# chechaohp/gan-ode

Measured on AMD Instinct MI355X. Metric: generated videos/sec (16-frame clips), higher is better.
Workload: dtype f32

## Files before the change

### gan-ode_amd/_lib.py

```python
from __future__ import annotations

import ctypes as C
import os

_HERE = os.path.dirname(os.path.abspath(__file__))
LIB_PATH = os.path.join(_HERE, "lib", "libgode.so")

i32, i64, f32, ptr = C.c_int32, C.c_int64, C.c_float, C.c_void_p
cint, u32, u64 = C.c_int, C.c_uint32, C.c_uint64

ACT_NONE, ACT_RELU, ACT_LRELU, ACT_TANH_OUT = 0, 1, 2, 3
EPI_RAW, EPI_TANH = 0, 1
FPROP, DGRAD = 0, 1
OP_IGEMM, OP_WGRAD, OP_BN_FINALIZE, OP_BN_BWD, OP_ODE_FWD, OP_ODE_BWD, OP_BCE, OP_ADAM, OP_PACK = range(1, 10)
OP_ODERNN_FWD, OP_ODERNN_BWD, OP_BN_APPLY, OP_COL2IM = 10, 11, 12, 13
OP_SDE_FWD, OP_SDE_BWD = 14, 15
OP_CDE_FWD, OP_CDE_BWD = 16, 17
OP_WGAN = 18
OP_GRU_FWD, OP_GRU_BWD = 19, 20
OP_DNOISE = 21
OP_CATEG, OP_CE = 22, 23
OP_CHSTATS, OP_CBN_EMBED, OP_CBN_EMBED_BWD, OP_CBN_APPLY, OP_CBN_BWD, OP_GRES_OUT, OP_GRES_OUT_BWD, OP_SN_FWD, OP_SN_BWD = range(24, 33)
REC_ADAM_NOISE = -1
ODE_NPARAM = 2672
ODERNN_NPARAM = 2176
SDE_NPARAM = 3216
CDE_NPARAM = 7536
CDE_MAX_N = 4096
# ... 4 lines not shown
class ConvGeom(C.Structure):
    _fields_ = [(n, i32) for n in "N Ci Co Di Hi Wi Do Ho Wo kd kh kw sd sh sw pd ph pw".split()]

    def key(self):
        return tuple(getattr(self, n) for n, _ in self._fields_)


class _Op(C.Structure):
    """An op of gode_run (a GODE_OPS row of gode.h): a subclass names its kind and its `int FN(const op*, stream)` entry
    point once; _STRUCTS, the prototypes, EXPORTS and run_one's dispatch all follow from the subclasses."""


class IgemmOp(_Op):
    _fields_ = [("g", ConvGeom), ("dir", i32), ("act", i32), ("epilogue", i32), ("tile", i32), ("src", ptr),
                ("wpack", ptr), ("out", ptr), ("scale", ptr), ("shift", ptr), ("stats", ptr), ("gs", i64 * 5),
                ("work", ptr), ("groups", i32), ("pad3_", i32)]
    KIND, FN = OP_IGEMM, "gode_igemm"


class WgradOp(_Op):
    _fields_ = [("g", ConvGeom), ("act", i32), ("xform_on_y", i32), ("splits", i32), ("accumulate", i32),
                ("x", ptr), ("y", ptr), ("scale", ptr), ("shift", ptr), ("work", ptr), ("dw", ptr),
                ("co_perm", ptr), ("co_canon", i64), ("xs", i64 * 5)]
    KIND, FN = OP_WGRAD, "gode_wgrad"


class BnFinalizeOp(_Op):
    _fields_ = [("stats", ptr), ("rows", i32), ("ncols", i32), ("C", i32), ("count", i64), ("gamma", ptr),
                ("beta", ptr), ("running_mean", ptr), ("running_var", ptr), ("num_batches_tracked", ptr),
                ("mean", ptr), ("invstd", ptr), ("scale", ptr), ("shift", ptr), ("momentum", f32), ("eps", f32),
                ("training", i32), ("pad_", i32), ("groups", i32), ("rows0", i32), ("nseg", i32), ("order", i32),
# ... 337 lines not shown
```

### gan-ode_amd/csrc/conv_geom.h

```cpp
#pragma once
#include <stdint.h>
#include "../../include/gode.h"

#if defined(__HIPCC__)
#define GODE_HD __host__ __device__ inline
#else
#define GODE_HD inline
#endif

#define GODE_MAX_PHASES 8

struct PhaseGeom {
  int32_t Md, Mh, Mw;
  int32_t M;
  int32_t Td, Th, Tw;
  int32_t K;
  int32_t Kp;
  int32_t Od, Oh, Ow;
  int32_t Pd, Ph, Pw;
  int32_t kd0, kh0, kw0;
  int32_t row0;
  int32_t img0;
  int64_t w_off;
};

struct IgemmGeom {
  int32_t nphase;
  int32_t Cg;
  int32_t Ncols;
  int32_t Sd, Sh, Sw;
  int32_t J;
  int32_t Gd, Gh, Gw;
  int32_t OSd, OSh, OSw;
  int32_t Xd, Xh, Xw;
  int32_t kstep_d, kstep_h, kstep_w;
  int32_t fullk;
  PhaseGeom ph[GODE_MAX_PHASES];
};

GODE_HD int gode_ceil_div(int a, int b) { return (a + b - 1) / b; }

inline int gode_build_igemm_geom(const gode_conv_geom& g, int dir, IgemmGeom* out) {
  IgemmGeom& G = *out;
  G.fullk = 0;
  if (g.N <= 0 || g.Ci <= 0 || g.Co <= 0) return GODE_E_SHAPE;
  if ((g.Di + 2 * g.pd - g.kd) / g.sd + 1 != g.Do || (g.Hi + 2 * g.ph - g.kh) / g.sh + 1 != g.Ho ||
      (g.Wi + 2 * g.pw - g.kw) / g.sw + 1 != g.Wo)
    return GODE_E_SHAPE;
  if (dir == GODE_FPROP) {
    G.nphase = 1; G.Cg = g.Ci; G.Ncols = g.Co;
    G.Sd = g.sd; G.Sh = g.sh; G.Sw = g.sw; G.J = 1;
    G.Gd = g.Di; G.Gh = g.Hi; G.Gw = g.Wi;
    G.OSd = G.OSh = G.OSw = 1;
    G.Xd = g.Do; G.Xh = g.Ho; G.Xw = g.Wo;
    G.kstep_d = G.kstep_h = G.kstep_w = 1;
    PhaseGeom& p = G.ph[0];
    p.Md = g.Do; p.Mh = g.Ho; p.Mw = g.Wo; p.M = g.N * p.Md * p.Mh * p.Mw;
    p.Td = g.kd; p.Th = g.kh; p.Tw = g.kw; p.K = p.Td * p.Th * p.Tw * G.Cg; p.Kp = (p.K + 3) & ~3;
    p.Od = -g.pd; p.Oh = -g.ph; p.Ow = -g.pw; p.Pd = p.Ph = p.Pw = 0;
    p.kd0 = p.kh0 = p.kw0 = 0; p.row0 = 0; p.img0 = 0; p.w_off = 0;
    return 0;
  }
  if (dir != GODE_DGRAD) return GODE_E_ARG;
  if (g.Do == 1 && g.Ho == 1 && g.Wo == 1 && g.pd == 0 && g.ph == 0 && g.pw == 0 && g.Di == g.kd &&
      g.Hi == g.kh && g.Wi == g.kw && g.kd * g.kh * g.kw > 1) {
    G.fullk = 1; G.nphase = 1; G.Cg = g.Co; G.Ncols = g.kd * g.kh * g.kw * g.Ci;
    G.Sd = G.Sh = G.Sw = 1; G.J = 1; G.Gd = G.Gh = G.Gw = 1;
    G.OSd = G.OSh = G.OSw = 1; G.Xd = G.Xh = G.Xw = 1;
    G.kstep_d = G.kstep_h = G.kstep_w = 1;
    PhaseGeom& p = G.ph[0];
    p.Md = p.Mh = p.Mw = 1; p.M = g.N; p.Td = p.Th = p.Tw = 1; p.K = G.Cg; p.Kp = (p.K + 3) & ~3;
    p.Od = p.Oh = p.Ow = 0; p.Pd = p.Ph = p.Pw = 0; p.kd0 = p.kh0 = p.kw0 = 0; p.row0 = 0; p.img0 = 0; p.w_off = 0;
    return 0;
  }
  if (g.sd * g.sh * g.sw > GODE_MAX_PHASES) return GODE_E_SHAPE;
  G.Cg = g.Co; G.Ncols = g.Ci;
  G.Sd = G.Sh = G.Sw = 1; G.J = -1;
  G.Gd = g.Do; G.Gh = g.Ho; G.Gw = g.Wo;
  G.OSd = g.sd; G.OSh = g.sh; G.OSw = g.sw;
  G.Xd = g.Di; G.Xh = g.Hi; G.Xw = g.Wi;
  G.kstep_d = g.sd; G.kstep_h = g.sh; G.kstep_w = g.sw;
  int np = 0; int64_t woff = 0;
  for (int fd = 0; fd < g.sd; ++fd)
    for (int fh = 0; fh < g.sh; ++fh)
      for (int fw = 0; fw < g.sw; ++fw) {
        PhaseGeom& p = G.ph[np++];
        const int phi[3] = {fd, fh, fw};
        const int X[3] = {g.Di, g.Hi, g.Wi}, s[3] = {g.sd, g.sh, g.sw}, k[3] = {g.kd, g.kh, g.kw},
                  pad[3] = {g.pd, g.ph, g.pw};
        int Mx[3], T[3], O[3], k0[3];
// ... 3 lines not shown
          k0[a] = r;
          T[a] = k[a] > r ? (k[a] - r + s[a] - 1) / s[a] : 0;
          O[a] = (phi[a] + pad[a] - r) / s[a];
        }
        p.Md = Mx[0]; p.Mh = Mx[1]; p.Mw = Mx[2]; p.M = g.N * Mx[0] * Mx[1] * Mx[2];
        p.Td = T[0]; p.Th = T[1]; p.Tw = T[2]; p.K = T[0] * T[1] * T[2] * G.Cg; p.Kp = (p.K + 3) & ~3;
        p.Od = O[0]; p.Oh = O[1]; p.Ow = O[2]; p.Pd = fd; p.Ph = fh; p.Pw = fw;
        p.kd0 = k0[0]; p.kh0 = k0[1]; p.kw0 = k0[2];
        p.row0 = 0; p.img0 = 0; p.w_off = woff;
        woff += (int64_t)G.Ncols * p.Kp;
      }
  G.nphase = np;
  return 0;
}

inline int64_t gode_pack_floats(const IgemmGeom& G) {
  int64_t t = 0;
  for (int i = 0; i < G.nphase; ++i) t += (int64_t)G.Ncols * G.ph[i].Kp;
  return t;
}

GODE_HD int64_t gode_w_index(const gode_conv_geom& g, int co, int ci, int kd, int kh, int kw) {
  return ((((int64_t)co * g.Ci + ci) * g.kd + kd) * g.kh + kh) * g.kw + kw;
}

GODE_HD int64_t gode_pack_source(const gode_conv_geom& g, int dir, const IgemmGeom& G, const PhaseGeom& p, int n,
                                 int k, const int32_t* co_perm) {
  if (k >= p.K) return -1;
  int co, ci, kd, kh, kw;
  if (G.fullk) {
    const int tapn = n / g.Ci;
    ci = n - tapn * g.Ci; co = k;
    kd = tapn / (g.kh * g.kw); kh = (tapn / g.kw) % g.kh; kw = tapn % g.kw;
// ... 12 lines not shown
```

### gan-ode_amd/csrc/igemm.hip

```cpp
#include <stdlib.h>
#include "common.h"
#include "conv_geom.h"

int gode_launch_conv_patch_fprop(const gode_igemm_op* op, const int64_t* gs, hipStream_t st);

struct IgemmArgs {
  IgemmGeom G;
  const float* src;
  const float* w;
  float* out;
  const float* scale;
  const float* shift;
  float* stats;
  int32_t gsN, gsD, gsH, gsW, gsC;
  int32_t act, epilogue;
  int32_t MB, NB, xcd_mode;
  int32_t tapskip, dmajor;
  int32_t stagger;
  int32_t ksplit, slabs_per_split;
  float* work;
  int32_t out_numel;
  int32_t stats_rows;
  uint32_t src_bytes, w_bytes;
};

__device__ __forceinline__ void igemm_block_id(const IgemmArgs& a, int& mblk, int& nblk, int& phase, int& split) {
  const int MB = a.MB, NC = a.NB * a.G.nphase;
  split = blockIdx.x / (MB * NC);
  const int id = blockIdx.x - split * (MB * NC);
  int combo;
  if (a.xcd_mode == 1) {
    const int x = id & 7, j = id >> 3;
    if ((NC & 7) == 0) { combo = x + 8 * (j / MB); mblk = j % MB; }
    else { const int parts = 8 / NC; combo = x % NC; mblk = j * parts + x / NC; }
  } else if (a.xcd_mode == 2) {
    const int x = id & 7, j = id >> 3;
    combo = j % NC; mblk = (j / NC) * 8 + x;
  } else if (a.xcd_mode == 3) {
    const int x = id & 7, j = id >> 3;
    combo = j % NC; mblk = x * (MB >> 3) + j / NC;
  } else {
// ... 952 lines not shown
      int k = (int)((1152 + t64 / 2) / t64);
      if (k < 1) k = 1;
      while (k > 1 && (min_slabs / k < 8 || out_bytes * k > 192e6)) --k;
      best_tile = TILE_64x64; best_k = k;
    }
  }
  *tile_out = best_tile;
  sp_out->positions = positions;
  sp_out->ksplit = 1; sp_out->slabs_per_split = 0;
  if (best_k > 1) {
    sp_out->slabs_per_split = gode_ceil_div(max_slabs, best_k);
    sp_out->ksplit = gode_ceil_div(max_slabs, sp_out->slabs_per_split);
  }
}

static int prepare(const gode_igemm_op* op, IgemmArgs* A, int* tile, int* max_mblk, int* rows, SplitPlan* sp, int* rows0 = nullptr) {
  int rc = gode_build_igemm_geom(op->g, op->dir, &A->G);
  if (rc) return rc;
  const bool grouped = op->groups == 2;
  if (grouped) {
    if (op->dir != GODE_FPROP || op->g.N % 2 != 0 || A->G.nphase != 1) return GODE_E_ARG;
    A->G.ph[1] = A->G.ph[0];
    A->G.ph[0].M /= 2; A->G.ph[1].M = A->G.ph[0].M; A->G.ph[1].img0 = op->g.N / 2;
    A->G.nphase = 2;
  } else if (op->groups != 0 && op->groups != 1) return GODE_E_ARG;
  static const char* menv = getenv("GODE_IGEMM_MODEL");
  static const bool sweeping = getenv("GODE_IGEMM_SWEEP") != nullptr;
  const char* fenv = sweeping ? getenv("GODE_IGEMM_FORCE") : nullptr;
  int ftile = 0, fk = 0;
  if (fenv && sscanf(fenv, "%d,%d", &ftile, &fk) == 2 && op->tile == 0 && fast_geometry(A->G) && A->G.Ncols > 4 &&
      strides_allow_vec(op, A->G)) {
    int max_slabs = 0;
    for (int i = 0; i < A->G.nphase; ++i) if ((A->G.ph[i].K >> 5) > max_slabs) max_slabs = A->G.ph[i].K >> 5;
    *tile = ftile;
    sp->positions = op->g.N * A->G.Xd * A->G.Xh * A->G.Xw; sp->ksplit = 1; sp->slabs_per_split = 0;
    if (fk > 1) { sp->slabs_per_split = gode_ceil_div(max_slabs, fk); sp->ksplit = gode_ceil_div(max_slabs, sp->slabs_per_split); }
  } else if (op->tile == 0 && fast_geometry(A->G) && A->G.Ncols > 4 && strides_allow_vec(op, A->G) && (!menv || atoi(menv) != 0)) {
    choose_fast(op, A->G, tile, sp);
  } else {
  *tile = pick_tile_split_aware(op->g, A->G, op->tile);
  *sp = plan_split(op, A->G, *tile);
  }
  if (grouped && sp->ksplit > 1 && (sp->positions / 2) % SPLITK_ROWS != 0) {
    sp->ksplit = 1; sp->slabs_per_split = 0;
  }
  const int bm = tile_bm(*tile);
  int r0 = 0, mx = 0;
  for (int i = 0; i < A->G.nphase; ++i) {
    A->G.ph[i].row0 = r0;
    const int mb = gode_ceil_div(A->G.ph[i].M, bm);
    r0 += mb;
    if (mb > mx) mx = mb;
  }
  *max_mblk = mx;
  *rows = sp->ksplit > 1 ? gode_ceil_div(sp->positions, SPLITK_ROWS) : r0;
  if (rows0) *rows0 = !grouped ? *rows : (sp->ksplit > 1 ? *rows / 2 : A->G.ph[1].row0);
// ... 1 lines not shown
}

extern "C" int gode_igemm_stats_rows0(const gode_igemm_op* op) {
  IgemmArgs A; int tile, mx, rows, rows0; SplitPlan sp;
  int rc = prepare(op, &A, &tile, &mx, &rows, &sp, &rows0);
  return rc ? rc : rows0;
}

extern "C" double gode_igemm_model_cycles(const gode_igemm_op* op) {
  if (!op || op->groups == 2 || op->tile != 0) return -1.0;
  IgemmArgs A;
  if (gode_build_igemm_geom(op->g, op->dir, &A.G)) return -1.0;
  static const char* menv = getenv("GODE_IGEMM_MODEL");
  if (!fast_geometry(A.G) || A.G.Ncols <= 4 || !strides_allow_vec(op, A.G) || (menv && atoi(menv) == 0)) return -1.0;
  int tile; SplitPlan sp; double cyc = -1.0;
  choose_fast(op, A.G, &tile, &sp, &cyc);
  return cyc;
}

extern "C" int gode_igemm_stats_segments(const gode_igemm_op* op, int32_t split_images, int32_t* seg) {
  if (!op || !seg || op->groups == 2 || split_images <= 0 || split_images >= op->g.N) return GODE_E_ARG;
  IgemmArgs A; int tile, mx, rows; SplitPlan sp;
  int rc = prepare(op, &A, &tile, &mx, &rows, &sp);
  if (rc) return rc;
  if (sp.ksplit > 1) {
    const int64_t per_img = (int64_t)A.G.Xd * A.G.Xh * A.G.Xw;
    const int64_t b = (int64_t)split_images * per_img;
    if (b % SPLITK_ROWS != 0) return GODE_E_SHAPE;
    seg[0] = 0; seg[1] = (int32_t)(b / SPLITK_ROWS); seg[2] = rows;
    return 1;
  }
  const int bm = tile_bm(tile);
  for (int i = 0; i < A.G.nphase; ++i) {
    const PhaseGeom& P = A.G.ph[i];
    const int64_t per_img = (int64_t)P.Md * P.Mh * P.Mw;
    const int64_t b = (int64_t)split_images * per_img;
// ... 36 lines not shown
    static const char* xenv = getenv("GODE_IGEMM_XCD");
    const int force = xenv ? atoi(xenv) : -1;
    const int64_t wbytes = gode_pack_floats(A.G) * 4;
    const bool ok1 = (NC % 8 == 0) || (NC < 8 && 8 % NC == 0 && MB % (8 / NC) == 0);
    const bool ok2 = MB % 8 == 0;
    const int64_t images = (int64_t)A.out_numel / ((int64_t)A.G.Xd * A.G.Xh * A.G.Xw * A.G.Ncols);
    const int64_t in_bytes = images * A.G.Gd * A.G.Gh * A.G.Gw * A.G.Cg * 4;
    int mode = ok2 ? (wbytes * 8 < 3 * in_bytes ? 3 : 0) : 0;
    if (A.dmajor > 0) mode = ok2 ? 2 : (ok1 ? 1 : 0);
    if (force == 0) mode = 0;
    if (force == 1 && ok1) mode = 1;
    if (force == 2 && ok2) mode = 2;
    if (force == 3 && ok2) mode = 3;
    A.xcd_mode = mode;
    dim3 g1(MB * NC * sp.ksplit);
    const bool has_xf = A.scale != nullptr || A.act != GODE_ACT_NONE;
    static const char* genv = getenv("GODE_IGEMM_GLDS");
    const bool glds = (genv ? atoi(genv) != 0 : true) && A.src_bytes != 0 && A.w_bytes != 0;
    if (!has_xf && glds && !double_buf) {
      if (A.tapskip) hipLaunchKernelGGL((igemm_fast_kernel<WM, WN, TM, TN, 3, false>), g1, block, 0, st, A);
      else hipLaunchKernelGGL((igemm_fast_kernel<WM, WN, TM, TN, 2, false>), g1, block, 0, st, A);
    } else if (double_buf) {
      if (has_xf) hipLaunchKernelGGL((igemm_fast_kernel<WM, WN, TM, TN, 1, true>), g1, block, 0, st, A);
      else hipLaunchKernelGGL((igemm_fast_kernel<WM, WN, TM, TN, 1, false>), g1, block, 0, st, A);
    } else {
      if (has_xf) hipLaunchKernelGGL((igemm_fast_kernel<WM, WN, TM, TN, 0, true>), g1, block, 0, st, A);
      else hipLaunchKernelGGL((igemm_fast_kernel<WM, WN, TM, TN, 0, false>), g1, block, 0, st, A);
    }
    if (sp.ksplit > 1) {
      GODE_LAUNCH_CHECK();
// ... 28 lines not shown
  }
  int64_t span = 1 + (int64_t)(op->g.N - 1) * gs[0] + (int64_t)(G.Gd - 1) * gs[1] + (int64_t)(G.Gh - 1) * gs[2] +
                 (int64_t)(G.Gw - 1) * gs[3] + (int64_t)(G.Cg - 1) * gs[4];
  int64_t outn = (int64_t)op->g.N * G.Xd * G.Xh * G.Xw * G.Ncols;
  for (int i = 0; i < 5; ++i) if (gs[i] < 0) return GODE_E_ARG;
  if (span >= (1ll << 31) || outn >= (1ll << 31)) return GODE_E_SHAPE;
  if (op->src && op->wpack && op->out && ((uintptr_t)op->wpack % 16) == 0) {
    const int pr = gode_launch_conv_patch_fprop(op, gs, (hipStream_t)stream);
    if (pr != 0) return pr < 0 ? pr : 0;
  }
  A.src = op->src; A.w = op->wpack; A.out = op->out; A.scale = op->scale; A.shift = op->shift; A.stats = op->stats;
  A.gsN = (int)gs[0]; A.gsD = (int)gs[1]; A.gsH = (int)gs[2]; A.gsW = (int)gs[3]; A.gsC = (int)gs[4];
  A.act = op->act; A.epilogue = op->epilogue;
  A.stagger = 0;
  A.dmajor = 0;
  A.tapskip = igemm_wants_tapskip(op, G);
  if (A.tapskip) A.dmajor = op->g.N;
  A.stats_rows = rows;
  A.src_bytes = span * 4 < (1ll << 31) ? (uint32_t)(span * 4) : 0u;
  A.w_bytes = gode_pack_floats(G) * 4 < (1ll << 31) ? (uint32_t)(gode_pack_floats(G) * 4) : 0u;
  A.work = op->work; A.out_numel = (int32_t)outn; A.ksplit = 1; A.slabs_per_split = 0; A.MB = 0; A.NB = 0; A.xcd_mode = 0;
  if ((op->scale == nullptr) != (op->shift == nullptr)) return GODE_E_ARG;
  const bool vec = gs[4] == 1 && (G.Cg % 4) == 0 && (gs[0] % 4) == 0 && (gs[1] % 4) == 0 && (gs[2] % 4) == 0 &&
                   (gs[3] % 4) == 0 && ((uintptr_t)op->src % 16) == 0 &&
                   (op->scale == nullptr || ((uintptr_t)op->scale % 16 == 0 && (uintptr_t)op->shift % 16 == 0));
  if (((uintptr_t)op->wpack % 16) != 0) return GODE_E_ARG;
  hipStream_t st = (hipStream_t)stream;
  if (op->groups != 2) {
    int maxM = 0, minK = 1 << 30; bool kp_ok = true;
    for (int i = 0; i < G.nphase; ++i) {
      if (G.ph[i].M > maxM) maxM = G.ph[i].M;
// ... 60 lines not shown
  const int32_t* co_perm;
};

__global__ void pack_kernel(const PackArgs a) {
  const PhaseGeom& P = a.G.ph[blockIdx.z];
  const int64_t total = (int64_t)a.G.Ncols * P.Kp;
  for (int64_t i = (int64_t)blockIdx.x * blockDim.x + threadIdx.x; i < total; i += (int64_t)gridDim.x * blockDim.x) {
    const int n = (int)(i / P.Kp), k = (int)(i - (int64_t)n * P.Kp);
    const int64_t src = gode_pack_source(a.g, a.dir, a.G, P, n, k, a.co_perm);
    a.wp[P.w_off + i] = src >= 0 ? a.w[src] : 0.f;
  }
}

extern "C" int64_t gode_pack_size(const gode_conv_geom* g, int dir) {
  IgemmGeom G;
  int rc = gode_build_igemm_geom(*g, dir, &G);
  return rc ? rc : gode_pack_floats(G);
}

#define PACK_BATCH 8
struct PackPhase { int32_t Th, Tw, K, Kp, kd0, kh0, kw0, pad_; int64_t w_off, total; };
struct PackEntry {
  const float* w; float* wp; const int32_t* co_perm;
  int32_t nphase, Cg, fullk, dir, ks_d, ks_h, ks_w, Ci, kd, kh, kw, Co;
  PackPhase ph[GODE_MAX_PHASES];
};
struct PackBatch { PackEntry e[PACK_BATCH]; };
static_assert(sizeof(PackBatch) <= 4096, "kernel-argument budget");

__global__ void __launch_bounds__(256) pack_batch_kernel(const PackBatch b) {
  const PackEntry& E = b.e[blockIdx.z];
  if ((int)blockIdx.y >= E.nphase) return;
  const PackPhase& P = E.ph[blockIdx.y];
  const int taps = E.kd * E.kh * E.kw;
  for (int64_t i = (int64_t)blockIdx.x * 256 + threadIdx.x; i < P.total; i += (int64_t)gridDim.x * 256) {
    const int n = (int)(i / P.Kp), k = (int)(i - (int64_t)n * P.Kp);
    float v = 0.f;
    if (k < P.K) {
      int co, ci, kd, kh, kw;
      if (E.fullk) {
// ... 42 lines not shown
    const int co_l = tid & (PACK_T - 1), ci_l = tid >> 4;
    for (int p = 0; p < E.nphase; ++p) {
      const PackPhase& P = E.ph[p];
      float* dst = E.wp + P.w_off + (int64_t)(ci0 + ci_l) * P.Kp + co0 + co_l;
      int j = 0;
      for (int kd = P.kd0; kd < E.kd; kd += E.ks_d)
        for (int kh = P.kh0; kh < E.kh; kh += E.ks_h)
          for (int kw = P.kw0; kw < E.kw; kw += E.ks_w, ++j) {
            const int t = (kd * E.kh + kh) * E.kw + kw;
            if (t >= t0 && t < t0 + TT) dst[(int64_t)j * E.Cg] = brick[co_l * CS + ci_l * 33 + (t - t0)];
          }
    }
  }
}

static bool pack_tileable(const PackEntry& E) {
  const int taps = E.kd * E.kh * E.kw;
  if (E.co_perm || E.fullk || taps < 4 || taps > 64 || (taps & (taps - 1)) != 0 || E.Ci % PACK_T != 0 || E.Co % PACK_T != 0) return false;
  for (int i = 0; i < E.nphase; ++i) if (E.ph[i].K != E.ph[i].Kp) return false;
  return true;
}

extern "C" int gode_pack_batch_(const gode_pack_op* const* ops, int n, void* stream) {
  for (int at = 0; at < n; at += PACK_BATCH) {
    PackBatch B;
    const int cnt = n - at < PACK_BATCH ? n - at : PACK_BATCH;
    int64_t mx = 0;
    for (int e = 0; e < cnt; ++e) {
      const gode_pack_op* op = ops[at + e];
      if (!op || !op->w || !op->wpack) return GODE_E_ARG;
      IgemmGeom G;
      const int rc = gode_build_igemm_geom(op->g, op->dir, &G);
      if (rc) return rc;
      PackEntry& E = B.e[e];
      E.w = op->w; E.wp = op->wpack; E.co_perm = op->co_perm;
      E.nphase = G.nphase; E.Cg = G.Cg; E.fullk = G.fullk; E.dir = op->dir;
      E.ks_d = G.kstep_d; E.ks_h = G.kstep_h; E.ks_w = G.kstep_w;
      E.Ci = op->g.Ci; E.kd = op->g.kd; E.kh = op->g.kh; E.kw = op->g.kw; E.Co = op->g.Co;
// ... 14 lines not shown
        const int taps = E.kd * E.kh * E.kw, TT = taps < 32 ? taps : 32;
        const int t = (E.Ci / PACK_T) * (E.Co / PACK_T) * (taps / TT);
        if (t > tiles) tiles = t;
        T.e[nt++] = E;
      } else {
        for (int i = 0; i < E.nphase; ++i) if (E.ph[i].total > mr) mr = E.ph[i].total;
        R.e[nr++] = E;
      }
    }
    if (nt > 0) {
      hipLaunchKernelGGL(pack_tile_kernel, dim3(tiles, 1, nt), dim3(256), 0, (hipStream_t)stream, T);
      GODE_LAUNCH_CHECK();
    }
    if (nr > 0 && mr > 0) {
      int blocks = (int)((mr + 1023) / 1024); if (blocks > 512) blocks = 512; if (blocks < 1) blocks = 1;
      hipLaunchKernelGGL(pack_batch_kernel, dim3(blocks, GODE_MAX_PHASES, nr), dim3(256), 0, (hipStream_t)stream, R);
      GODE_LAUNCH_CHECK();
    }
  }
  return 0;
}

extern "C" int gode_pack_weights(const gode_conv_geom* g, int dir, const float* w, float* wpack, const int32_t* co_perm,
                                 int32_t co_canon, void* stream) {
  (void)co_canon;
  if (!g || !w || !wpack) return GODE_E_ARG;
  PackArgs A;
  int rc = gode_build_igemm_geom(*g, dir, &A.G);
  if (rc) return rc;
  A.g = *g; A.dir = dir; A.w = w; A.wp = wpack; A.co_perm = co_perm;
  int64_t mx = 0;
  for (int i = 0; i < A.G.nphase; ++i) { int64_t t = (int64_t)A.G.Ncols * A.G.ph[i].Kp; if (t > mx) mx = t; }
  if (mx == 0) return 0;
  int blocks = (int)((mx + 255) / 256); if (blocks > 2048) blocks = 2048;
  hipLaunchKernelGGL(pack_kernel, dim3(blocks, 1, A.G.nphase), dim3(256), 0, (hipStream_t)stream, A);
  GODE_LAUNCH_CHECK();
  return 0;
}
```

### gan-ode_amd/engine.py

```python
from __future__ import annotations

import ctypes as C
from dataclasses import dataclass
from typing import List, Optional, Sequence

import numpy as np
import torch

from . import _lib as L


def make_geom(N, Ci, Co, xi, yo, k, s, p) -> L.ConvGeom:
    return L.ConvGeom(N, Ci, Co, xi[0], xi[1], xi[2], yo[0], yo[1], yo[2], k[0], k[1], k[2], s[0], s[1], s[2],
                      p[0], p[1], p[2])


def conv_out(i, k, s, p):
    return (i + 2 * p - k) // s + 1


def dptr(t: Optional[torch.Tensor]):
    return None if t is None else t.data_ptr()


# ... 64 lines not shown
        self.busy = False
        self.generation = 0
        self._fwd_training = True
        self.pack_cache = pack_cache if pack_cache is not None else {}
        lib = L.lib()
        f32 = dict(dtype=torch.float32, device=device)
        self.x_in = torch.zeros(specs[0].in_dims(), **f32) if owns_input else None
        self.x0n = torch.empty(specs[0].in_dims(), **f32) if specs[0].noise else None
        self.y = [torch.empty(s.out_dims(), **f32) for s in specs[:-1]]
        self.a = [torch.empty(s.out_dims(), **f32) if self._materialize(l) else None for l, s in enumerate(specs[:-1])]
        self.out_dims = specs[-1].out_dims()
        self.wpack_f, self.wpack_b = [], [None] * self.nl
        self.stats, self.stat_rows = [], []
        self.mean, self.invstd, self.scale, self.shift = [], [], [], []
        self._two_f, self._two_b, self._rows_ab = {}, {}, {}
        for l, s in enumerate(specs):
            n = lib.gode_pack_size(C.byref(s.geom), s.fwd_dir)
            if n <= 0:
                raise RuntimeError(f"bad geometry for pack ({n})")
            self.wpack_f.append(self._shared_pack(l, s.fwd_dir, n))
            C_out = s.out_dims()[4]
            two = self._two_f[l] = bool(self.split) and 0 < l < self.nl - 1 and self._two_launches(s.geom, s.fwd_dir)
            if s.has_bn:
                probe = L.IgemmOp(g=s.geom, dir=s.fwd_dir, tile=0, groups=groups)
                if two:
                    ra, rb = (lib.gode_igemm_stats_rows(C.byref(L.IgemmOp(g=self._part_geom(s.geom, n), dir=s.fwd_dir, tile=0)))
                              for n in (self.split, s.geom.N - self.split))
                    rows = ra + rb if ra > 0 and rb > 0 else -1
                    self._rows_ab[l] = (ra, rb)
                else:
                    rows = lib.gode_igemm_stats_rows(C.byref(probe))
                if rows <= 0:
                    raise RuntimeError(f"layer {l}: no partial-statistics layout for this geometry ({rows})")
                ncols = self._ncols(s)
                self.stat_rows.append(rows)
                self.stats.append(torch.empty(rows * 2 * ncols, **f32))
                ng = 2 if self._G2 else 1
                self.mean.append(torch.empty(ng * C_out, **f32)); self.invstd.append(torch.empty(ng * C_out, **f32))
                self.scale.append(torch.empty(ng * C_out, **f32)); self.shift.append(torch.empty(ng * C_out, **f32))
# ... 141 lines not shown
        return min(cost) > 0 and cost[1] + cost[2] + 12000.0 < cost[0]

    def _rank1_head(self, l, has_tanh):
        if l != self.nl - 1 or l == 0 or not has_tanh:
            return False
        s, g = self.specs[l], self.specs[l].geom
        return (s.fwd_dir == L.DGRAD and not s.has_bn and s.co_perm is None and self.specs[l - 1].has_bn and g.Ci == 1 and
                g.kd == g.kh == g.kw == 1 and g.sd == g.sh == g.sw == 1 and g.Di == g.Do == 1 and g.pd == 0 and
                g.ph == g.pw and g.Ho == g.Hi + 2 * g.ph and g.Wo == g.Wi + 2 * g.pw and self.params[l].weight.is_contiguous()
                and self.params[l].weight.data_ptr() % 16 == 0)

    def _half_geom(self, g):
        h = L.ConvGeom(*g.key())
        h.N = g.N // 2
        return h

    def _build_fwd(self, training: bool):
        ops = []
        packs = []
        patch = {}
        lib = L.lib()
        G2 = self.groups == 2
        noise = patch["noise"] = []
        if self.x0n is not None:
            n0, d0, h0, w0, c0 = self.specs[0].in_dims()
            ng = 2 if G2 else 1
            per = d0 * h0 * w0 * c0
            for k in range(ng):
                op = L.DnoiseOp(x=None, out=self.x0n.data_ptr() + 4 * k * (n0 // ng) * per, M=(n0 // ng) * d0 * h0 * w0,
                                C=c0, act=L.ACT_NONE, N=n0 // ng, D=d0, H=h0, W=w0, layer=0)
# ... 64 lines not shown
            if self._two_f.get(l):
                ra = self._rows_ab[l][0] if s.has_bn else 0
                per_in, per_out = int(np.prod(s.in_dims()[1:])), int(np.prod(s.out_dims()[1:]))
                for n, img0, st_off in ((self.split, 0, 0), (s.geom.N - self.split, self.split, ra * 2 * self._ncols(s))):
                    ops.append(L.IgemmOp(g=self._part_geom(s.geom, n), dir=s.fwd_dir, act=act, epilogue=s.epilogue, tile=0,
                                         src=src.data_ptr() + 4 * img0 * per_in, wpack=dptr(self.wpack_f[l]),
                                         out=self.y[l].data_ptr() + 4 * img0 * per_out, scale=dptr(sc), shift=dptr(sh),
                                         stats=self.stats[l].data_ptr() + 4 * st_off if want_stats else None, groups=0))
                op = None
            else:
                op = L.IgemmOp(g=s.geom, dir=s.fwd_dir, act=act, epilogue=s.epilogue, tile=0, src=dptr(src),
                               wpack=dptr(self.wpack_f[l]), out=dptr(self.y[l]) if l < self.nl - 1 else None,
                               scale=dptr(sc), shift=dptr(sh),
                               stats=dptr(self.stats[l]) if want_stats else None,
                               groups=2 if (G2 and s.has_bn) else 0)
                ops.append(op)
            if l == 0:
                patch["first"] = op
            if l == self.nl - 1:
                patch["last"] = op
            if s.has_bn:
                rows0 = lib.gode_igemm_stats_rows0(C.byref(op)) if G2 else 0
                fin = L.BnFinalizeOp(stats=dptr(self.stats[l]), rows=self.stat_rows[l], ncols=self._ncols(s),
                                     C=s.out_dims()[4], count=self._count(l) // self.groups, gamma=dptr(p.gamma),
                                     beta=dptr(p.beta), running_mean=dptr(p.running_mean),
                                     running_var=dptr(p.running_var),
                                     num_batches_tracked=dptr(p.num_batches_tracked), mean=dptr(self.mean[l]),
                                     invstd=dptr(self.invstd[l]), scale=dptr(self.scale[l]),
                                     shift=dptr(self.shift[l]), momentum=self.momentum, eps=self.eps,
                                     training=1 if training else 0, groups=self.groups if G2 else 0, rows0=rows0)
# ... 344 lines not shown
```

### include/gode.h

```cpp
#ifndef GODE_H
#define GODE_H
#include <stdint.h>
#ifdef __cplusplus
extern "C" {
#endif

#define GODE_VERSION 105

enum { GODE_OK = 0, GODE_E_ARG = -1, GODE_E_SHAPE = -2, GODE_E_KIND = -3 };
enum { GODE_ACT_NONE = 0, GODE_ACT_RELU = 1, GODE_ACT_LRELU = 2,
       GODE_ACT_TANH_OUT = 3  };
enum { GODE_EPI_RAW = 0, GODE_EPI_TANH = 1 };
enum { GODE_FPROP = 0, GODE_DGRAD = 1 };

typedef struct gode_conv_geom {
  int32_t N, Ci, Co;
  int32_t Di, Hi, Wi;
  int32_t Do, Ho, Wo;
  int32_t kd, kh, kw;
  int32_t sd, sh, sw;
  int32_t pd, ph, pw;
} gode_conv_geom;

typedef struct gode_igemm_op {
  gode_conv_geom g;
  int32_t dir, act, epilogue, tile;
  const float* src;
  const float* wpack;
  float* out;
  const float* scale;
  const float* shift;
  float* stats;
  int64_t gs[5];
  float* work;
  int32_t groups, pad3_;
} gode_igemm_op;
int gode_igemm(const gode_igemm_op* op, void* stream);
int64_t gode_igemm_work_size(const gode_igemm_op* op);
int gode_igemm_stats_rows(const gode_igemm_op* op);
int gode_igemm_stats_rows0(const gode_igemm_op* op);
int gode_igemm_stats_segments(const gode_igemm_op* op, int32_t split_images, int32_t* seg);
double gode_igemm_model_cycles(const gode_igemm_op* op);
int64_t gode_pack_size(const gode_conv_geom* g, int dir);
int gode_pack_weights(const gode_conv_geom* g, int dir, const float* w, float* wpack, const int32_t* co_perm,
                      int32_t co_canon, void* stream);

typedef struct gode_wgrad_op {
  gode_conv_geom g;
  int32_t act, xform_on_y, splits, accumulate;
  const float* x;
// ... 320 lines not shown
  X(CATEG,         22, gode_categ_op,         gode_categ_onehot)  \
  X(CE,            23, gode_ce_op,            gode_ce_logits)     \
  X(CHSTATS,       24, gode_chstats_op,       gode_chstats)       \
  X(CBN_EMBED,     25, gode_cbn_embed_op,     gode_cbn_embed)     \
  X(CBN_EMBED_BWD, 26, gode_cbn_embed_bwd_op, gode_cbn_embed_bwd) \
  X(CBN_APPLY,     27, gode_cbn_apply_op,     gode_cbn_apply)     \
  X(CBN_BWD,       28, gode_cbn_bwd_op,       gode_cbn_bwd)       \
  X(GRES_OUT,      29, gode_gres_out_op,      gode_gres_out)      \
  X(GRES_OUT_BWD,  30, gode_gres_out_bwd_op,  gode_gres_out_bwd)  \
  X(SN_FWD,        31, gode_sn_op,            gode_sn_fwd)        \
  X(SN_BWD,        32, gode_sn_bwd_op,        gode_sn_bwd)
#define GODE_ENUM_ROW_(name, value, op_t, fn) GODE_OP_##name = value,
enum { GODE_OPS(GODE_ENUM_ROW_) GODE_OP_PACK = 9 };
#undef GODE_ENUM_ROW_
typedef struct gode_pack_op {
  gode_conv_geom g; int32_t dir, co_canon; const float* w; float* wpack; const int32_t* co_perm;
} gode_pack_op;
int gode_run(const int32_t* kinds, const void* const* ops, int32_t n, void* stream);

int gode_version(void);
int gode_sizeof(int kind);

#ifdef __cplusplus
}
#endif
#endif
```

Measured before the change: 35410.

## Split transposed-conv phases into border sub-phases that skip out-of-range taps

For dgrad (transposed-conv) layers, each stride phase is divided into runs of output positions whose valid kernel-tap range matches, so interior sub-phases use the full tap set and border sub-phases use trimmed K. Per-sub-phase weights are packed into extra regions, and a tile table maps blocks to sub-phases in a single launch. The aim is to stop multiplying padded or zero taps at borders. In exchange it adds more phases, a per-block table search, a cost model that picks when to use it, and larger packed weights.

```diff
diff --git a/gan-ode_amd/_lib.py b/gan-ode_amd/_lib.py
--- a/gan-ode_amd/_lib.py
+++ b/gan-ode_amd/_lib.py
@@ -12,6 +12,7 @@
 ACT_NONE, ACT_RELU, ACT_LRELU, ACT_TANH_OUT = 0, 1, 2, 3
 EPI_RAW, EPI_TANH = 0, 1
 FPROP, DGRAD = 0, 1
+PACK_BORDER = 0x100
 OP_IGEMM, OP_WGRAD, OP_BN_FINALIZE, OP_BN_BWD, OP_ODE_FWD, OP_ODE_BWD, OP_BCE, OP_ADAM, OP_PACK = range(1, 10)
 OP_ODERNN_FWD, OP_ODERNN_BWD, OP_BN_APPLY, OP_COL2IM = 10, 11, 12, 13
 OP_SDE_FWD, OP_SDE_BWD = 14, 15
@@ -46,7 +47,7 @@
 class IgemmOp(_Op):
     _fields_ = [("g", ConvGeom), ("dir", i32), ("act", i32), ("epilogue", i32), ("tile", i32), ("src", ptr),
                 ("wpack", ptr), ("out", ptr), ("scale", ptr), ("shift", ptr), ("stats", ptr), ("gs", i64 * 5),
-                ("work", ptr), ("groups", i32), ("pad3_", i32)]
+                ("work", ptr), ("groups", i32), ("border", i32)]
     KIND, FN = OP_IGEMM, "gode_igemm"
 
 
diff --git a/gan-ode_amd/csrc/conv_geom.h b/gan-ode_amd/csrc/conv_geom.h
--- a/gan-ode_amd/csrc/conv_geom.h
+++ b/gan-ode_amd/csrc/conv_geom.h
@@ -8,7 +8,8 @@
 #define GODE_HD inline
 #endif
 
-#define GODE_MAX_PHASES 8
+#define GODE_MAX_PHASES 16
+#define GODE_MAX_STRIDE_PHASES 8
 
 struct PhaseGeom {
   int32_t Md, Mh, Mw;
@@ -34,6 +35,7 @@
   int32_t OSd, OSh, OSw;
   int32_t Xd, Xh, Xw;
   int32_t kstep_d, kstep_h, kstep_w;
+  int32_t border;
   int32_t fullk;
   PhaseGeom ph[GODE_MAX_PHASES];
 };
@@ -42,7 +44,7 @@
 
 inline int gode_build_igemm_geom(const gode_conv_geom& g, int dir, IgemmGeom* out) {
   IgemmGeom& G = *out;
-  G.fullk = 0;
+  G.fullk = 0; G.border = 0;
   if (g.N <= 0 || g.Ci <= 0 || g.Co <= 0) return GODE_E_SHAPE;
   if ((g.Di + 2 * g.pd - g.kd) / g.sd + 1 != g.Do || (g.Hi + 2 * g.ph - g.kh) / g.sh + 1 != g.Ho ||
       (g.Wi + 2 * g.pw - g.kw) / g.sw + 1 != g.Wo)
@@ -73,7 +75,7 @@
     p.Od = p.Oh = p.Ow = 0; p.Pd = p.Ph = p.Pw = 0; p.kd0 = p.kh0 = p.kw0 = 0; p.row0 = 0; p.img0 = 0; p.w_off = 0;
     return 0;
   }
-  if (g.sd * g.sh * g.sw > GODE_MAX_PHASES) return GODE_E_SHAPE;
+  if (g.sd * g.sh * g.sw > GODE_MAX_STRIDE_PHASES) return GODE_E_SHAPE;
   G.Cg = g.Co; G.Ncols = g.Ci;
   G.Sd = G.Sh = G.Sw = 1; G.J = -1;
   G.Gd = g.Do; G.Gh = g.Ho; G.Gw = g.Wo;
@@ -107,9 +109,71 @@
   return 0;
 }
 
+inline int gode_build_igemm_geom_border(const gode_conv_geom& g, int dir, IgemmGeom* out) {
+  IgemmGeom P0;
+  int rc = gode_build_igemm_geom(g, dir, &P0);
+  *out = P0;
+  if (rc || dir != GODE_DGRAD || P0.fullk) return rc;
+  IgemmGeom B = P0;
+  const int S[3] = {P0.Sd, P0.Sh, P0.Sw}, Gx[3] = {P0.Gd, P0.Gh, P0.Gw}, OS[3] = {P0.OSd, P0.OSh, P0.OSw},
+            ks[3] = {P0.kstep_d, P0.kstep_h, P0.kstep_w};
+  struct Run { int a, len, lo, hi; };
+  int np = 0;
+  int64_t woff = 0;
+  for (int i = 0; i < P0.nphase; ++i) woff += (int64_t)P0.Ncols * P0.ph[i].Kp;
+  for (int i = 0; i < P0.nphase; ++i) {
+    const PhaseGeom& p = P0.ph[i];
+    const int Mx[3] = {p.Md, p.Mh, p.Mw}, T[3] = {p.Td, p.Th, p.Tw}, O[3] = {p.Od, p.Oh, p.Ow};
+    Run runs[3][GODE_MAX_PHASES];
+    int nr[3] = {0, 0, 0};
+    for (int a = 0; a < 3; ++a) {
+      if (Mx[a] <= 0 || T[a] <= 0) return 0;
+      for (int q = 0; q < Mx[a]; ++q) {
+        const int c = q * S[a] + O[a];
+        int lo = c - Gx[a] + 1, hi = c;
+        if (lo < 0) lo = 0;
+        if (hi > T[a] - 1) hi = T[a] - 1;
+        if (lo > hi) return 0;
+        if (nr[a] > 0 && runs[a][nr[a] - 1].lo == lo && runs[a][nr[a] - 1].hi == hi) { ++runs[a][nr[a] - 1].len; continue; }
+        if (nr[a] == GODE_MAX_PHASES) return 0;
+        runs[a][nr[a]++] = Run{q, 1, lo, hi};
+      }
+    }
+    if ((int64_t)np + (int64_t)nr[0] * nr[1] * nr[2] > GODE_MAX_PHASES) return 0;
+    for (int rd = 0; rd < nr[0]; ++rd)
+      for (int rh = 0; rh < nr[1]; ++rh)
+        for (int rw = 0; rw < nr[2]; ++rw) {
+          const Run* r[3] = {&runs[0][rd], &runs[1][rh], &runs[2][rw]};
+          PhaseGeom& s = B.ph[np++];
+          s = p;
+          s.Md = r[0]->len; s.Mh = r[1]->len; s.Mw = r[2]->len; s.M = g.N * s.Md * s.Mh * s.Mw;
+          s.Td = r[0]->hi - r[0]->lo + 1; s.Th = r[1]->hi - r[1]->lo + 1; s.Tw = r[2]->hi - r[2]->lo + 1;
+          s.K = s.Td * s.Th * s.Tw * P0.Cg; s.Kp = (s.K + 3) & ~3;
+          s.Od = O[0] + r[0]->a * S[0] + P0.J * r[0]->lo; s.Oh = O[1] + r[1]->a * S[1] + P0.J * r[1]->lo;
+          s.Ow = O[2] + r[2]->a * S[2] + P0.J * r[2]->lo;
+          s.Pd = p.Pd + r[0]->a * OS[0]; s.Ph = p.Ph + r[1]->a * OS[1]; s.Pw = p.Pw + r[2]->a * OS[2];
+          s.kd0 = p.kd0 + r[0]->lo * ks[0]; s.kh0 = p.kh0 + r[1]->lo * ks[1]; s.kw0 = p.kw0 + r[2]->lo * ks[2];
+          if (s.Td == p.Td && s.Th == p.Th && s.Tw == p.Tw) s.w_off = p.w_off;
+          else { s.w_off = woff; woff += (int64_t)P0.Ncols * s.Kp; }
+        }
+  }
+  for (int i = 1; i < np; ++i) {
+    const PhaseGeom t = B.ph[i];
+    int j = i;
+    while (j > 0 && B.ph[j - 1].K < t.K) { B.ph[j] = B.ph[j - 1]; --j; }
+    B.ph[j] = t;
+  }
+  B.nphase = np; B.border = 1;
+  *out = B;
+  return 0;
+}
+
 inline int64_t gode_pack_floats(const IgemmGeom& G) {
   int64_t t = 0;
-  for (int i = 0; i < G.nphase; ++i) t += (int64_t)G.Ncols * G.ph[i].Kp;
+  for (int i = 0; i < G.nphase; ++i) {
+    const int64_t e = G.ph[i].w_off + (int64_t)G.Ncols * G.ph[i].Kp;
+    if (e > t) t = e;
+  }
   return t;
 }
 
diff --git a/gan-ode_amd/csrc/igemm.hip b/gan-ode_amd/csrc/igemm.hip
--- a/gan-ode_amd/csrc/igemm.hip
+++ b/gan-ode_amd/csrc/igemm.hip
@@ -22,9 +22,22 @@
   int32_t out_numel;
   int32_t stats_rows;
   uint32_t src_bytes, w_bytes;
+  int32_t ntab;
+  int32_t tile0[GODE_MAX_PHASES + 1];
 };
 
 __device__ __forceinline__ void igemm_block_id(const IgemmArgs& a, int& mblk, int& nblk, int& phase, int& split) {
+  if (a.ntab > 0) {
+    const int id = blockIdx.x;
+    int p = 0;
+    while (p + 1 < a.ntab && id >= a.tile0[p + 1]) ++p;
+    const int t = id - a.tile0[p], NB = a.NB, mb = (a.tile0[p + 1] - a.tile0[p]) / NB;
+    const int grp = t / (8 * NB), r = t - grp * 8 * NB, rest = mb - grp * 8;
+    if (rest >= 8) { mblk = grp * 8 + (r & 7); nblk = r >> 3; }
+    else { mblk = grp * 8 + r % rest; nblk = r / rest; }
+    phase = p; split = 0;
+    return;
+  }
   const int MB = a.MB, NC = a.NB * a.G.nphase;
   split = blockIdx.x / (MB * NC);
   const int id = blockIdx.x - split * (MB * NC);
@@ -1007,9 +1020,47 @@
   }
 }
 
-static int prepare(const gode_igemm_op* op, IgemmArgs* A, int* tile, int* max_mblk, int* rows, SplitPlan* sp, int* rows0 = nullptr) {
+static bool border_table(const gode_igemm_op* op, const IgemmGeom& G, IgemmGeom* B) {
+  if (!op->border || op->dir != GODE_DGRAD || op->groups == 2 || G.fullk || igemm_wants_tapskip(op, G)) return false;
+  return gode_build_igemm_geom_border(op->g, op->dir, B) == 0 && B->border != 0;
+}
+
+#define BORDER_LOSS 1.06
+static void choose_border(const gode_igemm_op* op, const IgemmGeom& B, int* tile_out, double* cycles_out) {
+  (void)op;
+  static const int tiles[4] = {TILE_128x128, TILE_128x64, TILE_64x64, TILE_256x128};
+  double best = 1e300; int best_tile = TILE_128x64;
+  for (int ti = 0; ti < 4; ++ti) {
+    const int t = tiles[ti], bm = tile_bm(t), bn = tile_bn(t);
+    if (bn >= 2 * B.Ncols && bn > 32) continue;
+    if (t != TILE_128x64 && t != TILE_64x64) continue;
+    const double cps = t == TILE_256x128 ? 8192.0 : (t == TILE_128x128 ? 4096.0 : (t == TILE_128x64 ? 2048.0 : 1024.0));
+    const int resident = t == TILE_256x128 ? 1 : (t == TILE_128x128 ? 2 : (t == TILE_128x64 ? 3 : 4));
+    const double eff2 = t == TILE_64x64 ? 0.70 : (t == TILE_256x128 ? 0.785 : 0.76);
+    int64_t ntiles = 0; int max_slabs = 0;
+    for (int i = 0; i < B.nphase; ++i) {
+      ntiles += (int64_t)gode_ceil_div(B.ph[i].M, bm) * gode_ceil_div(B.Ncols, bn);
+      if ((B.ph[i].K >> 5) > max_slabs) max_slabs = B.ph[i].K >> 5;
+    }
+    if (3 * ntiles < 4 * 256 * (int64_t)resident) continue;
+    const double eff = (resident >= 2 || t == TILE_256x128) ? eff2 : 0.8 * eff2;
+    double work = 0;
+    for (int i = 0; i < B.nphase; ++i)
+      work += (double)gode_ceil_div(B.ph[i].M, bm) * gode_ceil_div(B.Ncols, bn) * (4000.0 + (B.ph[i].K >> 5) * cps / eff);
+    const double cyc = BORDER_LOSS * work / 256.0;
+    if (cyc < best) { best = cyc; best_tile = t; }
+  }
+  *tile_out = best_tile; *cycles_out = best;
+}
+
+static int prepare(const gode_igemm_op* op, IgemmArgs* A, int* tile, int* max_mblk, int* rows, SplitPlan* sp, int* rows0 = nullptr,
+                   double* cycles = nullptr) {
   int rc = gode_build_igemm_geom(op->g, op->dir, &A->G);
   if (rc) return rc;
+  A->ntab = 0;
+  if (cycles) *cycles = -1.0;
+  IgemmGeom B;
+  const bool can_border = border_table(op, A->G, &B);
   const bool grouped = op->groups == 2;
   if (grouped) {
     if (op->dir != GODE_FPROP || op->g.N % 2 != 0 || A->G.nphase != 1) return GODE_E_ARG;
@@ -1028,11 +1079,24 @@
     *tile = ftile;
     sp->positions = op->g.N * A->G.Xd * A->G.Xh * A->G.Xw; sp->ksplit = 1; sp->slabs_per_split = 0;
     if (fk > 1) { sp->slabs_per_split = gode_ceil_div(max_slabs, fk); sp->ksplit = gode_ceil_div(max_slabs, sp->slabs_per_split); }
+    if (can_border && fk <= 1) A->G = B;
   } else if (op->tile == 0 && fast_geometry(A->G) && A->G.Ncols > 4 && strides_allow_vec(op, A->G) && (!menv || atoi(menv) != 0)) {
-    choose_fast(op, A->G, tile, sp);
+    double cyc = -1.0;
+    choose_fast(op, A->G, tile, sp, &cyc);
+    if (can_border && fast_geometry(B) && sp->ksplit == 1) {
+      int tb; double cb;
+      choose_border(op, B, &tb, &cb);
+      if (cb < 0.97 * cyc) { A->G = B; *tile = tb; sp->ksplit = 1; sp->slabs_per_split = 0; cyc = cb; }
+    }
+    if (cycles) *cycles = cyc;
   } else {
-  *tile = pick_tile_split_aware(op->g, A->G, op->tile);
-  *sp = plan_split(op, A->G, *tile);
+    *tile = pick_tile_split_aware(op->g, A->G, op->tile);
+    *sp = plan_split(op, A->G, *tile);
+    if (can_border && sp->ksplit == 1 && op->tile != 0) {
+      const int tb = pick_tile_split_aware(op->g, B, op->tile);
+      const SplitPlan sb = plan_split(op, B, tb);
+      if (sb.ksplit == 1) { A->G = B; *tile = tb; *sp = sb; }
+    }
   }
   if (grouped && sp->ksplit > 1 && (sp->positions / 2) % SPLITK_ROWS != 0) {
     sp->ksplit = 1; sp->slabs_per_split = 0;
@@ -1064,12 +1128,18 @@
   static const char* menv = getenv("GODE_IGEMM_MODEL");
   if (!fast_geometry(A.G) || A.G.Ncols <= 4 || !strides_allow_vec(op, A.G) || (menv && atoi(menv) == 0)) return -1.0;
   int tile; SplitPlan sp; double cyc = -1.0;
+  IgemmGeom B;
   choose_fast(op, A.G, &tile, &sp, &cyc);
+  if (sp.ksplit == 1 && border_table(op, A.G, &B) && fast_geometry(B)) {
+    double cb;
+    choose_border(op, B, &tile, &cb);
+    if (cb < 0.97 * cyc) cyc = cb;
+  }
   return cyc;
 }
 
 extern "C" int gode_igemm_stats_segments(const gode_igemm_op* op, int32_t split_images, int32_t* seg) {
-  if (!op || !seg || op->groups == 2 || split_images <= 0 || split_images >= op->g.N) return GODE_E_ARG;
+  if (!op || !seg || op->groups == 2 || op->border || split_images <= 0 || split_images >= op->g.N) return GODE_E_ARG;
   IgemmArgs A; int tile, mx, rows; SplitPlan sp;
   int rc = prepare(op, &A, &tile, &mx, &rows, &sp);
   if (rc) return rc;
@@ -1136,6 +1206,14 @@
     if (force == 3 && ok2) mode = 3;
     A.xcd_mode = mode;
     dim3 g1(MB * NC * sp.ksplit);
+    if (A.G.border) {
+      if (sp.ksplit > 1 || A.tapskip) return GODE_E_ARG;
+      constexpr int BM = WM * TM * 32;
+      A.ntab = A.G.nphase; A.tile0[0] = 0;
+      for (int i = 0; i < A.G.nphase; ++i) A.tile0[i + 1] = A.tile0[i] + gode_ceil_div(A.G.ph[i].M, BM) * NB;
+      for (int i = A.G.nphase + 1; i <= GODE_MAX_PHASES; ++i) A.tile0[i] = A.tile0[A.G.nphase];
+      g1 = dim3(A.tile0[A.G.nphase]);
+    }
     const bool has_xf = A.scale != nullptr || A.act != GODE_ACT_NONE;
     static const char* genv = getenv("GODE_IGEMM_GLDS");
     const bool glds = (genv ? atoi(genv) != 0 : true) && A.src_bytes != 0 && A.w_bytes != 0;
@@ -1194,7 +1272,7 @@
   A.act = op->act; A.epilogue = op->epilogue;
   A.stagger = 0;
   A.dmajor = 0;
-  A.tapskip = igemm_wants_tapskip(op, G);
+  A.tapskip = !G.border && igemm_wants_tapskip(op, G);
   if (A.tapskip) A.dmajor = op->g.N;
   A.stats_rows = rows;
   A.src_bytes = span * 4 < (1ll << 31) ? (uint32_t)(span * 4) : 0u;
@@ -1285,7 +1363,7 @@
 
 extern "C" int64_t gode_pack_size(const gode_conv_geom* g, int dir) {
   IgemmGeom G;
-  int rc = gode_build_igemm_geom(*g, dir, &G);
+  int rc = (dir & GODE_PACK_BORDER) ? gode_build_igemm_geom_border(*g, dir & ~GODE_PACK_BORDER, &G) : gode_build_igemm_geom(*g, dir, &G);
   return rc ? rc : gode_pack_floats(G);
 }
 
@@ -1294,7 +1372,7 @@
 struct PackEntry {
   const float* w; float* wp; const int32_t* co_perm;
   int32_t nphase, Cg, fullk, dir, ks_d, ks_h, ks_w, Ci, kd, kh, kw, Co;
-  PackPhase ph[GODE_MAX_PHASES];
+  PackPhase ph[GODE_MAX_STRIDE_PHASES];
 };
 struct PackBatch { PackEntry e[PACK_BATCH]; };
 static_assert(sizeof(PackBatch) <= 4096, "kernel-argument budget");
@@ -1367,6 +1445,8 @@
   }
 }
 
+static int gode_pack_batch_plain(const gode_pack_op* const* ops, int n, void* stream);
+
 static bool pack_tileable(const PackEntry& E) {
   const int taps = E.kd * E.kh * E.kw;
   if (E.co_perm || E.fullk || taps < 4 || taps > 64 || (taps & (taps - 1)) != 0 || E.Ci % PACK_T != 0 || E.Co % PACK_T != 0) return false;
@@ -1374,7 +1454,31 @@
   return true;
 }
 
-extern "C" int gode_pack_batch_(const gode_pack_op* const* ops, int n, void* stream) {
+static int pack_one(const gode_conv_geom* g, int dir, int border, const float* w, float* wpack, const int32_t* co_perm, void* stream);
+
+extern "C" int gode_pack_batch_(const gode_pack_op* const* all_ops, int n_all, void* stream) {
+  const gode_pack_op* plain[64];
+  int n = 0;
+  for (int i = 0; i <= n_all; ++i) {
+    const gode_pack_op* op = i < n_all ? all_ops[i] : nullptr;
+    if (i < n_all && !op) return GODE_E_ARG;
+    if (op && (op->dir & GODE_PACK_BORDER)) {
+      if (!op->w || !op->wpack) return GODE_E_ARG;
+      const int rc = pack_one(&op->g, op->dir & ~GODE_PACK_BORDER, 1, op->w, op->wpack, op->co_perm, stream);
+      if (rc) return rc;
+      continue;
+    }
+    if (op) plain[n++] = op;
+    if (n == 64 || (!op && n > 0)) {
+      const int rc = gode_pack_batch_plain(plain, n, stream);
+      if (rc) return rc;
+      n = 0;
+    }
+  }
+  return 0;
+}
+
+static int gode_pack_batch_plain(const gode_pack_op* const* ops, int n, void* stream) {
   for (int at = 0; at < n; at += PACK_BATCH) {
     PackBatch B;
     const int cnt = n - at < PACK_BATCH ? n - at : PACK_BATCH;
@@ -1419,7 +1523,7 @@
     }
     if (nr > 0 && mr > 0) {
       int blocks = (int)((mr + 1023) / 1024); if (blocks > 512) blocks = 512; if (blocks < 1) blocks = 1;
-      hipLaunchKernelGGL(pack_batch_kernel, dim3(blocks, GODE_MAX_PHASES, nr), dim3(256), 0, (hipStream_t)stream, R);
+      hipLaunchKernelGGL(pack_batch_kernel, dim3(blocks, GODE_MAX_STRIDE_PHASES, nr), dim3(256), 0, (hipStream_t)stream, R);
       GODE_LAUNCH_CHECK();
     }
   }
@@ -1430,8 +1534,24 @@
                                  int32_t co_canon, void* stream) {
   (void)co_canon;
   if (!g || !w || !wpack) return GODE_E_ARG;
+  return pack_one(g, dir & ~GODE_PACK_BORDER, (dir & GODE_PACK_BORDER) != 0, w, wpack, co_perm, stream);
+}
+
+static int pack_one(const gode_conv_geom* g, int dir, int border, const float* w, float* wpack, const int32_t* co_perm, void* stream) {
   PackArgs A;
-  int rc = gode_build_igemm_geom(*g, dir, &A.G);
+  if (border) {
+    int rc = pack_one(g, dir, 0, w, wpack, co_perm, stream);
+    if (rc) return rc;
+    rc = gode_build_igemm_geom_border(*g, dir, &A.G);
+    if (rc) return rc;
+    if (!A.G.border) return 0;
+    int np = 0;
+    for (int i = 0; i < A.G.nphase; ++i)
+      if (A.G.ph[i].w_off >= gode_pack_size(g, dir)) A.G.ph[np++] = A.G.ph[i];
+    A.G.nphase = np;
+    if (np == 0) return 0;
+  }
+  int rc = border ? 0 : gode_build_igemm_geom(*g, dir, &A.G);
   if (rc) return rc;
   A.g = *g; A.dir = dir; A.w = w; A.wp = wpack; A.co_perm = co_perm;
   int64_t mx = 0;
diff --git a/gan-ode_amd/engine.py b/gan-ode_amd/engine.py
--- a/gan-ode_amd/engine.py
+++ b/gan-ode_amd/engine.py
@@ -1,6 +1,7 @@
 from __future__ import annotations
 
 import ctypes as C
+import os
 from dataclasses import dataclass
 from typing import List, Optional, Sequence
 
@@ -102,15 +103,17 @@
         self.stats, self.stat_rows = [], []
         self.mean, self.invstd, self.scale, self.shift = [], [], [], []
         self._two_f, self._two_b, self._rows_ab = {}, {}, {}
+        self._border = self._border_layers() if os.environ.get("GODE_BORDER_SPLIT", "1") != "0" else {}
         for l, s in enumerate(specs):
-            n = lib.gode_pack_size(C.byref(s.geom), s.fwd_dir)
+            bord = l in self._border
+            n = lib.gode_pack_size(C.byref(s.geom), s.fwd_dir | (L.PACK_BORDER if bord else 0))
             if n <= 0:
                 raise RuntimeError(f"bad geometry for pack ({n})")
-            self.wpack_f.append(self._shared_pack(l, s.fwd_dir, n))
+            self.wpack_f.append(self._shared_pack(l, "border" if bord else s.fwd_dir, n))
             C_out = s.out_dims()[4]
             two = self._two_f[l] = bool(self.split) and 0 < l < self.nl - 1 and self._two_launches(s.geom, s.fwd_dir)
             if s.has_bn:
-                probe = L.IgemmOp(g=s.geom, dir=s.fwd_dir, tile=0, groups=groups)
+                probe = L.IgemmOp(g=s.geom, dir=s.fwd_dir, tile=0, groups=groups, border=1 if bord else 0)
                 if two:
                     ra, rb = (lib.gode_igemm_stats_rows(C.byref(L.IgemmOp(g=self._part_geom(s.geom, n), dir=s.fwd_dir, tile=0)))
                               for n in (self.split, s.geom.N - self.split))
@@ -282,6 +285,19 @@
         h = L.ConvGeom(*g.key())
         h.N = g.N // 2
         return h
+
+    def _border_layers(self):
+        if self.groups != 1 or self.split or self.noisy:
+            return {}
+        lib, out = L.lib(), {}
+        for l, s in enumerate(self.specs):
+            if s.fwd_dir != L.DGRAD or self._head_as_gemm(l) is not None:
+                continue
+            n = lib.gode_pack_size(C.byref(s.geom), L.DGRAD | L.PACK_BORDER)
+            if n <= lib.gode_pack_size(C.byref(s.geom), L.DGRAD):
+                continue
+            out[l] = n
+        return out
 
     def _build_fwd(self, training: bool):
         ops = []
@@ -376,6 +392,10 @@
                                scale=dptr(sc), shift=dptr(sh),
                                stats=dptr(self.stats[l]) if want_stats else None,
                                groups=2 if (G2 and s.has_bn) else 0)
+                if l in self._border:
+                    packs[-1] = (l, "border", L.PackOp(g=s.geom, dir=L.DGRAD | L.PACK_BORDER, co_canon=0, w=dptr(p.weight),
+                                                       wpack=dptr(self.wpack_f[l]), co_perm=dptr(s.co_perm)))
+                    op.border = 1
                 ops.append(op)
             if l == 0:
                 patch["first"] = op
diff --git a/include/gode.h b/include/gode.h
--- a/include/gode.h
+++ b/include/gode.h
@@ -12,6 +12,7 @@
        GODE_ACT_TANH_OUT = 3  };
 enum { GODE_EPI_RAW = 0, GODE_EPI_TANH = 1 };
 enum { GODE_FPROP = 0, GODE_DGRAD = 1 };
+enum { GODE_PACK_BORDER = 0x100 };
 
 typedef struct gode_conv_geom {
   int32_t N, Ci, Co;
@@ -33,7 +34,8 @@
   float* stats;
   int64_t gs[5];
   float* work;
-  int32_t groups, pad3_;
+  int32_t groups;
+  int32_t border;
 } gode_igemm_op;
 int gode_igemm(const gode_igemm_op* op, void* stream);
 int64_t gode_igemm_work_size(const gode_igemm_op* op);
@@ -384,7 +386,7 @@
 enum { GODE_OPS(GODE_ENUM_ROW_) GODE_OP_PACK = 9 };
 #undef GODE_ENUM_ROW_
 typedef struct gode_pack_op {
-  gode_conv_geom g; int32_t dir, co_canon; const float* w; float* wpack; const int32_t* co_perm;
+  gode_conv_geom g; int32_t dir , co_canon; const float* w; float* wpack; const int32_t* co_perm;
 } gode_pack_op;
 int gode_run(const int32_t* kinds, const void* const* ops, int32_t n, void* stream);
 
```

Result: faster. 37100, median of 6 (+4.8%).
